# reedrosenbluth/oscen

Hardware: AMD Instinct MI355X
Metric: voices*samples/sec (fm-synth graph, 48 kHz) (higher is better)
Workload: dtype f32

## Files before the change

oscen_amd/csrc/og_cluster.cpp:

```cpp
#include "og_engine.h"

#include <dlfcn.h>
#include <rccl/rccl.h>

#include <condition_variable>
#include <functional>
#include <mutex>
#include <thread>

__global__ void og_bus_accumulate(float* __restrict__ dst, const float* __restrict__ src, size_t n)
{
    const size_t i = (size_t)blockIdx.x * blockDim.x + threadIdx.x;
    if (i < n) dst[i] += src[i];
}

namespace {

struct Rccl {
    void* lib = nullptr;
    ncclResult_t (*CommInitAll)(ncclComm_t*, int, const int*) = nullptr;
    ncclResult_t (*CommDestroy)(ncclComm_t) = nullptr;
    ncclResult_t (*Reduce)(const void*, void*, size_t, ncclDataType_t, ncclRedOp_t, int, ncclComm_t, hipStream_t) = nullptr;
    ncclResult_t (*GroupStart)() = nullptr;
    ncclResult_t (*GroupEnd)() = nullptr;
// ... 373 lines not shown
                    HIPCK(hipStreamWaitEvent(e->stream, free_ev, 0));
                    for (size_t g = 0; g < nf; g += block) {
                        const uint32_t frames = (uint32_t)std::min<size_t>(block, nf - g);
                        e->process_async(frames, buf + g * vc);
                    }
                    e->flush_bus();
                    HIPCK(hipEventRecord(done, e->stream));
                });
            }
            wait_all();
            reduce_and_hand_over(b, nf);
            if (have_prev) {
                HIPCK(hipEventSynchronize(host_ready[b ^ 1]));
                memcpy(out + prev_f0 * channels, h_pin[b ^ 1], prev_nf * channels * sizeof(float));
            }
            have_prev = true;
            prev_f0 = f0;
            prev_nf = nf;
        }
        if (have_prev) {
            HIPCK(hipSetDevice(devs[0]));
            HIPCK(hipEventSynchronize(host_ready[b ^ 1]));
            memcpy(out + prev_f0 * channels, h_pin[b ^ 1], prev_nf * channels * sizeof(float));
        }
        sync_all();
    }
};

extern "C" {

int og_cluster_create(const og_graph_desc* g, uint64_t n_voices_total, const int* device_ids, uint32_t n_shards, og_cluster** out)
{
    if (!g || !device_ids || !out) return set_err(OG_E_INVALID, "null argument");
    if (n_shards == 0 || n_voices_total < n_shards) return set_err(OG_E_INVALID, "need at least one voice per shard");
    return guard([&] {
        std::unique_ptr<og_cluster> c(new og_cluster);
        c->total = n_voices_total;
        for (uint32_t s = 0; s <= n_shards; ++s) c->lo.push_back(n_voices_total * s / n_shards);
        for (uint32_t s = 0; s < n_shards; ++s) {
            const uint64_t nv = c->lo[s + 1] - c->lo[s];
            if (nv > 0xFFFFFFFFull) throw std::runtime_error("more than 2^32 voices in one shard");
            og_engine* raw = nullptr;
            const int rc = og_create(g, (uint32_t)nv, device_ids[s], &raw);
            if (rc != OG_OK) {
                if (rc == OG_E_DEVICE) throw HipError(og_last_error());
                throw std::runtime_error(og_last_error());
            }
            std::unique_ptr<og_engine> e(raw);
            if (e->cg->bus_stage == ogc::BusStage::Convolver)
                throw ogabi::Unsupported("a cluster over a graph with a post-mix Convolver is not supported in this version (the convolver runs on one device's bus)");
            e->bus_stage = false;
            {
                HIPCK(hipSetDevice(e->device));
                e->alloc_bus_buffers(e->auto_batch());
                e->bus_batch = e->auto_batch();
            }
            c->shard.push_back(e.get());
            e.release();
            int di = -1;
            for (size_t d = 0; d < c->devs.size(); ++d)
                if (c->devs[d] == device_ids[s]) di = (int)d;
            if (di < 0) {
                c->devs.push_back(device_ids[s]);
                di = (int)c->devs.size() - 1;
            }
            c->dev_of_shard.push_back(di);
            c->workers.emplace_back(new Worker);
        }
        c->channels = c->shard[0]->cg->channels;
        c->vch = c->shard[0]->cg->voice_channels;
        c->tremolo = c->shard[0]->cg->bus_stage == ogc::BusStage::Tremolo;
        const size_t nd = c->devs.size();
        c->dev_stream.assign(nd, nullptr);
        for (int b = 0; b < 2; ++b) {
            c->sh_buf[b].assign(n_shards, nullptr);
            c->sh_done[b].assign(n_shards, nullptr);
            c->dev_free[b].assign(nd, nullptr);
            c->dev_acc[b].assign(nd, nullptr);
        }
        for (size_t d = 0; d < nd; ++d) {
            HIPCK(hipSetDevice(c->devs[d]));
            HIPCK(hipStreamCreateWithFlags(&c->dev_stream[d], hipStreamNonBlocking));
            for (int b = 0; b < 2; ++b) {
                HIPCK(hipEventCreateWithFlags(&c->dev_free[b][d], hipEventDisableTiming));
                HIPCK(hipEventRecord(c->dev_free[b][d], c->dev_stream[d]));
            }
        }
        for (uint32_t s = 0; s < n_shards; ++s) {
            HIPCK(hipSetDevice(c->shard[s]->device));
            for (int b = 0; b < 2; ++b) HIPCK(hipEventCreateWithFlags(&c->sh_done[b][s], hipEventDisableTiming));
        }
        HIPCK(hipSetDevice(c->devs[0]));
        if (c->tremolo) {
            HIPCK(hipMalloc(&c->d_phase, 4));
            HIPCK(hipMemset(c->d_phase, 0, 4));
        }
        const char* force = ogabi::experiment_knob("OSCEN_GPU_FORCE_RCCL");
        if (nd > 1 || (force && atoi(force) != 0)) {
            Rccl& R = rccl();
            R.load();
            c->comms.assign(nd, nullptr);
            R.ck(R.CommInitAll(c->comms.data(), (int)nd, c->devs.data()), "ncclCommInitAll");
            c->use_rccl = true;
        }
        *out = c.release();
        return OG_OK;
    });
}
// ... 270 lines not shown
```

oscen_amd/csrc/og_engine.cpp:

```cpp
#include "og_engine.h"
#include "og_math.h"
#include "og_bus_conv.hip.h"
#include "og_asset_resample.hip.h"

#define OG_RED_SLICES 64
#define OG_RED_FRAMES 16
static_assert(OG_RED_FRAMES == OG_BUS_CHUNK, "og_bus_reduce reads the chunks og::bus_chunk_reduce writes");
#define OG_RED_GROUP 1024
__device__ __forceinline__ void og_bus_reduce_body(const float* __restrict__ partials, uint32_t n_rows, uint32_t frames,
                                                   float* __restrict__ out, uint32_t out_stride, uint32_t out_off)
{
    __shared__ float part[OG_RED_SLICES][OG_RED_FRAMES];
    __shared__ float quad[OG_RED_SLICES / 4][OG_RED_FRAMES];
    const uint32_t fx = threadIdx.x % OG_RED_FRAMES;
    const uint32_t slice = threadIdx.x / OG_RED_FRAMES;
    const uint32_t f = blockIdx.x * OG_RED_FRAMES + fx;
    const uint32_t row0 = blockIdx.y * OG_RED_GROUP;
    const uint32_t row1 = min(n_rows, row0 + OG_RED_GROUP);
    float acc[8] = {0.0f, 0.0f, 0.0f, 0.0f, 0.0f, 0.0f, 0.0f, 0.0f};
    const float* __restrict__ chunk = partials + (size_t)blockIdx.x * n_rows * OG_RED_FRAMES;
    if (f < frames) {
        uint32_t r = row0 + slice;
        for (; r + 7 * OG_RED_SLICES < row1; r += 8 * OG_RED_SLICES) {
#pragma unroll
// ... 127 lines not shown
    }
    return code;
}
int set_error(int code, const char* m) noexcept
{
    try {
        g_err.assign(m ? m : "");
    } catch (...) {
        g_err.clear();
    }
    return code;
}
}

namespace {
struct DeviceScratch {
    float* p = nullptr;
    explicit DeviceScratch(size_t floats) { HIPCK(hipMalloc(&p, std::max<size_t>(floats, 1) * 4)); }
    ~DeviceScratch() { if (p) (void)hipFree(p); }
    DeviceScratch(const DeviceScratch&) = delete;
    DeviceScratch& operator=(const DeviceScratch&) = delete;
};
std::map<std::string, std::shared_ptr<const SampleData>>& sample_registry()
{
    static std::map<std::string, std::shared_ptr<const SampleData>> R;
    return R;
}
std::mutex& sample_registry_lock()
{
    static std::mutex m;
    return m;
}
}
std::shared_ptr<const SampleData> lookup_sample(const std::string& name)
{
    std::lock_guard<std::mutex> lk(sample_registry_lock());
    auto it = sample_registry().find(name);
    return it == sample_registry().end() ? nullptr : it->second;
}
namespace {
void map_sample_channels(const SampleData& s, uint32_t width, float* dst)
{
    for (size_t t = 0; t < s.frames; ++t)
        for (uint32_t c = 0; c < width; ++c) {
            const uint32_t sc = s.channels == 1 ? 0u : std::min(c, s.channels - 1u);
            dst[t * width + c] = s.interleaved[t * s.channels + sc];
        }
}
}

void og_engine::conv_alloc(size_t need_hist)
{
    const size_t vc = cg->voice_channels;
    const size_t max_frames = (size_t)OG_MAX_BLOCK * batch_cap;
    const size_t keep = std::max(hist_keep, (std::max<size_t>(need_hist, 1) + OG_CONV_S - 1) / OG_CONV_S * OG_CONV_S);
    const size_t len = 2 * keep + 2 * max_frames;
    if (!d_hist || keep != hist_keep || len != hist_len) {
        float* n = nullptr;
        HIPCK(hipMalloc(&n, len * vc * 4));
        HIPCK(hipMemsetAsync(n, 0, len * vc * 4, stream));
        if (d_hist) {
            HIPCK(hipMemcpyAsync(n + (keep - hist_keep) * vc, d_hist + (hist_pos - hist_keep) * vc, hist_keep * vc * 4, hipMemcpyDeviceToDevice, stream));
            HIPCK(hipStreamSynchronize(stream));
            HIPCK(hipFree(d_hist));
        }
        d_hist = n;
        hist_keep = keep;
        hist_len = len;
        hist_pos = keep;
    }
    const uint32_t stride = (uint32_t)((max_frames + 3) / 4 * 4);
    const size_t half = (keep / OG_CONV_S + 1) * vc * stride;
    if (!d_conv_rows || stride != conv_row_stride || half != conv_rows_half) {
        if (d_conv_rows) HIPCK(hipFree(d_conv_rows));
        d_conv_rows = nullptr;
        HIPCK(hipMalloc(&d_conv_rows, 2 * half * 4));
        conv_row_stride = stride;
        conv_rows_half = half;
    }
    HIPCK(hipStreamSynchronize(stream));
}

std::shared_ptr<og_engine::ConvIR> og_engine::conv_build_asset(const std::string& name, const ogc::IrAsset& a)
{
    const uint32_t rate = graph_rate("og_set_bus_ir");
    const bool conform = a.rate != rate;
    const OgResamplePlan plan = conform ? og_resample_plan(a.frames, a.rate, rate) : OgResamplePlan{};
    const uint64_t K = conform ? plan.out_len : a.frames;
    if (K > OG_CONV_MAX_TAPS)
        throw ogabi::Unsupported("impulse response '" + name + "' (" + std::to_string(a.frames) + " frames at " + std::to_string(a.rate) + " Hz) has " +
                                 std::to_string(K) + " taps per channel once conformed to " + std::to_string(rate) + " Hz (at most " + std::to_string(OG_CONV_MAX_TAPS) + ")");
    if (K == 0)
        throw ogabi::Error(OG_E_INVALID, "impulse response '" + name + "' (" + std::to_string(a.frames) + " frames at " + std::to_string(a.rate) + " Hz) is empty once conformed to " + std::to_string(rate) + " Hz");
    const uint32_t vc = cg->voice_channels;
    const bool downmix = vc == 1 && a.channels > 1;
    auto ir = std::make_shared<ConvIR>();
    ir->planes = (a.channels == 1 || vc == 1) ? 1u : vc;
    ir->taps.resize((size_t)ir->planes * K);
    DeviceScratch d_src(a.interleaved.size()), d_conf(conform ? (size_t)K * a.channels : 1);
    bounce.h2d(d_src.p, a.interleaved.data(), a.interleaved.size() * 4, stream);
    if (conform) og_resample_launch(d_src.p, a.frames, a.channels, plan, d_conf.p, stream);
    HIPCK(hipMalloc(&ir->d, ir->taps.size() * 4));
    conv_bufs.push_back(ir->d);
    hipLaunchKernelGGL(og_bus_ir_planes, dim3((unsigned)((K + 255) / 256), ir->planes), dim3(256), 0, stream, conform ? d_conf.p : d_src.p, (uint32_t)K,
                       a.channels, downmix ? 1u : 0u, 1.0f / (float)a.channels, ir->d);
    HIPCK(hipGetLastError());
    bounce.d2h(ir->taps.data(), ir->d, ir->taps.size() * 4, stream);
// ... 175 lines not shown
    }
    TlEvent* sev = h_stage_ev[r];
    uint32_t* upd = h_stage_upd[r];
    const EventTimeline::Batch b = tl.plan_incremental(sev, upd, consumed_horizon(), launch_end());
    if (!b) return false;
    if (b.n_upd == 0) return true;
    HostProf::Scope pc(prof, HostProf::EV_COMMIT);
    tl.commit_incremental(b, sev, upd);
    static_assert(sizeof(OgEvent) == sizeof(uint4), "og_apply_event_updates copies events as 16-byte words");
    const uint32_t n_wg_upd = (uint32_t)((std::max(b.n_upd, b.n_ev) + 255) / 256);
    hipLaunchKernelGGL(og_apply_event_updates, dim3(n_wg_upd), dim3(256), 0, stream, (const uint4*)sev, (uint32_t)b.n_ev,
                       (uint4*)(d_events + b.base), (const uint32_t*)upd, (uint32_t)b.n_upd, d_ev_cursor, d_ev_end);
    HIPCK(hipGetLastError());
    stage_seq[r] = flush_seq + 1;
    batch_staged = true;
    stage_head = (stage_head + 1) % EV_RING;
    return true;
}

void og_engine::upload_events()
{
    if (!tl.needs_upload(launch_end())) return;
    EventTimeline::HoldLocal hold(tl);
    if (!tl.needs_upload(launch_end())) return;
    HostProf::Scope ps(prof, HostProf::SYNC_EVENTS);
    const bool bulk = tl.wants_rebuild() || tl.n_pending() > tl.stage_events() || tl.n_pending() > (size_t)V / 2 + 64 || !d_events;
    if (bulk || !incremental_update()) full_rebuild();
}

bool og_engine::rcp_cover(uint32_t need)
{
    if (need > rcp_cap) return false;
    if (need <= rcp_n) return true;
    const uint32_t n = std::min(rcp_cap, std::max(need, 2 * rcp_n));
    float* t = nullptr;
    HIPCK(hipMalloc(&t, ((size_t)OG_RCP_PAD + n + 1) * sizeof(float)));
    const uint32_t words = OG_RCP_PAD + n + 1;
    hipLaunchKernelGGL(og::rcp_table_fill<0>, dim3((words + 255) / 256), dim3(256), 0, stream, t, n);
    HIPCK(hipGetLastError());
    if (d_rcp) rcp_old.push_back(d_rcp);
    d_rcp = t;
    rcp_n = n;
    return true;
}

void og_engine::alloc_bus_buffers(uint32_t batch)
{
    HIPCK(hipStreamSynchronize(stream));
    for (float** p : {&d_partials, &d_partials2, &d_mono, &d_stage_bus})
        if (*p) {
            HIPCK(hipFree(*p));
            *p = nullptr;
        }
    batch_cap = batch;
    const size_t max_frames = (size_t)OG_MAX_BLOCK * batch;
    const size_t vc = cg->voice_channels;
    HIPCK(hipMalloc(&d_partials, (size_t)n_wg * max_frames * 4 * vc));
    HIPCK(hipMemset(d_partials, 0, (size_t)n_wg * max_frames * 4 * vc));
    HIPCK(hipMalloc(&d_partials2, ((size_t)n_wg / OG_RED_GROUP + 2 + 64) * max_frames * 4));
    HIPCK(hipMalloc(&d_stage_bus, max_frames * OG_MAX_BUS_CHANNELS * 4));
    if (cg->bus_stage == ogc::BusStage::Tremolo) HIPCK(hipMalloc(&d_mono, max_frames * 4));
    if (cg->bus_stage == ogc::BusStage::Convolver) conv_alloc(std::max(conv.cur ? conv.cur->K() : 0u, conv.old ? conv.old->K() : 0u));
    const size_t rows = (size_t)(cg->n_ramps + cg->n_streams);
    for (int i = 0; i < RAMP_RING && rows; ++i) {
        if (d_ramp[i]) HIPCK(hipFree(d_ramp[i]));
        if (h_ramp[i]) HIPCK(hipHostFree(h_ramp[i]));
        d_ramp[i] = h_ramp[i] = nullptr;
        HIPCK(hipMalloc(&d_ramp[i], rows * max_frames * 4));
        HIPCK(hipHostMalloc((void**)&h_ramp[i], rows * max_frames * 4, hipHostMallocDefault));
        ramp_seq[i] = 0;
    }
}

void og_engine::process_async(uint32_t frames, float* d_out)
{
    HIPCK(hipSetDevice(device));
    tl.drop_late_local(frame_now + frames);
    if (!queue.empty() && tl.n_pending() > std::min<size_t>(tl.stage_events() / 2, (size_t)V / 4 + 32)) flush_bus();
    if (queue.empty()) {
        q_frame0 = frame_now;
        q_frames = 0;
        q_ramps = cg->n_streams > 0;
        q_ramp_slot = -1;
    }
    const size_t stride = (size_t)OG_MAX_BLOCK * batch_cap;
    const bool ramping = active_ramps > 0 && cg->n_ramps > 0;
    if ((ramping || cg->n_streams > 0 || q_ramps) && cg->n_ramps + cg->n_streams > 0) {
        if (q_ramp_slot < 0) {
            q_ramp_slot = ramp_head;
            ramp_head = (ramp_head + 1) % RAMP_RING;
            batch_done(ramp_seq[q_ramp_slot]);
            float* tab0 = h_ramp[q_ramp_slot];
            for (size_t i = 0; i < cg->inputs.size(); ++i) {
                const int row = cg->inputs[i].ramp_row;
                if (row >= 0) std::fill(tab0 + (size_t)row * stride, tab0 + (size_t)row * stride + q_frames, ramps[i].current);
            }
        }
        q_ramps = true;
        float* tab = h_ramp[q_ramp_slot];
        for (uint32_t f = 0; f < frames; ++f) {
            for (size_t i = 0; i < cg->inputs.size(); ++i) {
                const int row = cg->inputs[i].ramp_row;
                if (row < 0) continue;
                if (active_ramps > 0 && ramps[i].tick()) active_ramps -= 1;
                tab[(size_t)row * stride + q_frames + f] = ramps[i].current;
            }
        }
        for (size_t i = 0; i < cg->inputs.size(); ++i) {
            if (cg->inputs[i].ramp_row >= 0) values[i] = ramps[i].current;
            const int srow = cg->inputs[i].stream_row;
            for (int k = 0; srow >= 0 && k < std::max(1, cg->inputs[i].decl.channels); ++k)
                memcpy(tab + (size_t)(srow + k) * stride + q_frames, stream_blocks[i].data() + (size_t)k * OG_MAX_BLOCK, (size_t)frames * 4);
        }
    }
    QueuedBlock qb;
    qb.dst = d_out ? d_out : d_bus;
    qb.frames = frames;
    qb.trem_rate = qb.trem_depth = 0.0f;
    qb.conv = 0;
    if (conv_on()) {
        if (conv.old && frame_now >= conv.fade_start + conv_fade_len()) conv_retire(conv.old);
        if (conv_pending) {
            conv_retire(conv.old);
            conv.old = conv.cur;
            conv.old_from = conv.cur_from;
            conv.cur = conv_pending;
            conv.cur_from = conv.fade_start = frame_now;
            conv_pending.reset();
        }
        if (q_conv.empty() || !q_conv.back().same(conv)) q_conv.push_back(conv);
        qb.conv = (uint32_t)q_conv.size() - 1;
    }
    if (cg->bus_stage == ogc::BusStage::Tremolo && bus_stage) {
        ogc::UEnv ev = env();
        qb.trem_rate = cg->tremolo_rate(ev);
        qb.trem_depth = cg->tremolo_depth(ev);
    }
    queue.push_back(qb);
    q_frames += frames;
    frame_now += frames;
    last_frames = frames;
    const bool ramps_done = ramping && active_ramps == 0 && cg->n_streams == 0;
    if (queue.size() >= bus_batch || n_taps > 0 || ramps_done) flush_bus();
}

void og_engine::flush_bus()
{
    if (queue.empty()) return;
    upload_events();
    HostProf::Scope ps(prof, HostProf::LAUNCH);
    OgBlockArgs A;
    memset(&A, 0, sizeof A);
    A.n_voices = V;
    A.frames = q_frames;
    A.ramp_stride = (uint32_t)((size_t)OG_MAX_BLOCK * batch_cap);
    A.lanes = lanes;
    A.split = split;
    A.wide = wide ? 1u : 0u;
    A.frame0 = q_frame0;
    A.state = d_state;
    A.lane_state = d_lane_state;
    A.lane_dump = d_lane_state ? d_lane_state + cg->lane_state.size() * (size_t)V * cg->lpv * cg->lane_width : nullptr;
    A.events = d_events;
    A.ev_end = d_ev_end;
    A.ev_cursor = d_ev_cursor;
    A.partials = d_partials;
    const uint32_t n_chunks16 = (q_frames + OG_RED_FRAMES - 1) / OG_RED_FRAMES;
    A.partial_plane = (uint32_t)((size_t)n_chunks16 * n_wg * OG_RED_FRAMES);
    A.taps = d_taps;
    A.tap_slot = d_tap_slot;
    A.out_ev = d_out_ev;
    A.out_ev_cap = out_ev_cap;
    A.out_ev_count = d_out_ev ? d_out_ev_count : nullptr;
    A.ev_lost = d_out_ev_count ? d_out_ev_count + 1 : nullptr;
    for (size_t k = 0; k < cg->rings.size(); ++k) {
        A.rings[k] = d_ring[k];
        A.ring_cap[k] = ring_cap[k];
    }
    {
        ogc::UEnv e = env();
        uint32_t starts[OG_MAX_LAUNCH_BLOCKS + 1];
        uint32_t acc = 0, nb = 0;
        for (const QueuedBlock& qb : queue) {
            if (nb < OG_MAX_LAUNCH_BLOCKS) starts[nb++] = acc;
            acc += qb.frames;
        }
        e.block_starts = starts;
        e.n_blocks = nb;
        for (const auto& up : cg->uprogs) A.slots[up.dst] = up.fn(e);
    }
    if (cg->player_slot0 >= 0) {
        uint32_t* ps = A.slots + cg->player_slot0;
        ps[0] = (uint32_t)((uintptr_t)d_pool & 0xFFFFFFFFu);
        ps[1] = (uint32_t)((uint64_t)(uintptr_t)d_pool >> 32);
        ps[2] = (uint32_t)((uintptr_t)d_desc & 0xFFFFFFFFu);
        ps[3] = (uint32_t)((uint64_t)(uintptr_t)d_desc >> 32);
        ps[4] = sample_cap;
    }
    if (rcp_cover(release_need(A.slots))) {
        A.rcp_tab = d_rcp;
        A.rcp_len = rcp_n;
    }
    const bool ramps_on = q_ramps && q_ramp_slot >= 0;
    if (ramps_on) {
        const int r = q_ramp_slot;
        const size_t rows = (size_t)(cg->n_ramps + cg->n_streams);
        HIPCK(hipMemcpyAsync(d_ramp[r], h_ramp[r], rows * A.ramp_stride * 4, hipMemcpyHostToDevice, stream));
        ramp_seq[r] = flush_seq + 1;
// ... 1125 lines not shown
    e->tl.reserve_pending(n);
    for (uint32_t i = 0; i < n; ++i)
        e->tl.push(e->phys(voices[i]), std::max(abs_frames[i], e->frame_now), target, values[i], false);
    return OG_OK;
    });
}

int og_process_block_async(og_engine* e, uint32_t frames, float* d_out_bus)
{
    if (!e) return set_err(OG_E_INVALID, "null engine");
    if (!e->inited) return set_err(OG_E_STATE, "og_init must be called before processing");
    if (frames > OG_MAX_BLOCK_SIZE) return set_err(OG_E_INVALID, "frames must be in 0..512");
    return guard([&] {
        if (frames == 0) {
            HIPCK(hipSetDevice(e->device));
            e->flush_bus();
            e->tl.drop_late_local(e->frame_now);
            e->last_frames = 0;
            return OG_OK;
        }
        e->process_async(frames, d_out_bus);
        return OG_OK;
    });
}

int og_process_blocks_async(og_engine* e, uint32_t frames, uint32_t n_blocks, float* d_out_bus, size_t out_stride_bytes)
{
    if (!e) return set_err(OG_E_INVALID, "null engine");
    if (!e->inited) return set_err(OG_E_STATE, "og_init must be called before processing");
    if (frames == 0 || frames > OG_MAX_BLOCK_SIZE) return set_err(OG_E_INVALID, "frames must be in 1..512");
    if (d_out_bus && out_stride_bytes % sizeof(float)) return set_err(OG_E_INVALID, "out_stride_bytes must be a multiple of 4");
    return guard([&] {
        for (uint32_t b = 0; b < n_blocks; ++b)
            e->process_async(frames, d_out_bus ? d_out_bus + (size_t)b * (out_stride_bytes / sizeof(float)) : nullptr);
        return OG_OK;
    });
}

int og_synchronize(og_engine* e)
{
    if (!e) return set_err(OG_E_INVALID, "null engine");
    return guard([&] {
        HIPCK(hipSetDevice(e->device));
        e->flush_bus();
        HIPCK(hipStreamSynchronize(e->stream));
        e->sync_lost_counter();
        return OG_OK;
    });
}

int og_set_bus_batching(og_engine* e, uint32_t blocks)
{
    if (!e) return set_err(OG_E_INVALID, "null engine");
    if (blocks > OG_MAX_LAUNCH_BLOCKS) return set_err(OG_E_INVALID, "bus batching: 0 (automatic) or 1..32 blocks");
    if (blocks == 0) blocks = e->auto_batch();
    return guard([&] {
        HIPCK(hipSetDevice(e->device));
        e->flush_bus();
        if (blocks > e->batch_cap) e->alloc_bus_buffers(blocks);
        e->bus_batch = blocks;
        return OG_OK;
    });
}

int og_flush(og_engine* e)
{
    if (!e) return set_err(OG_E_INVALID, "null engine");
    return guard([&] {
        HIPCK(hipSetDevice(e->device));
        e->flush_bus();
        return OG_OK;
    });
}

int og_process_block(og_engine* e, uint32_t frames, float* out_bus)
{
    if (!e) return set_err(OG_E_INVALID, "null engine");
    if (!e->inited) return set_err(OG_E_STATE, "og_init must be called before processing");
    if (frames > OG_MAX_BLOCK_SIZE) return set_err(OG_E_INVALID, "frames must be in 0..512");
    if (frames == 0 || !out_bus || e->n_taps > 0 || e->blocking_memcpy) {
        int rc = og_process_block_async(e, frames, nullptr);
        if (rc) return rc;
        return guard([&] {
            e->flush_bus();
            if (out_bus && frames)
                e->bounce.d2h(out_bus, e->d_bus, (size_t)frames * e->cg->channels * 4, e->stream);
            HIPCK(hipStreamSynchronize(e->stream));
            return OG_OK;
        });
    }
    return guard([&] {
        HIPCK(hipSetDevice(e->device));
        e->flush_bus();
        if (!e->h_bus_pinned) HIPCK(hipHostMalloc((void**)&e->h_bus_pinned, (size_t)OG_MAX_BLOCK * OG_MAX_BUS_CHANNELS * 4, hipHostMallocDefault));
        e->batch_staged = true;
        const uint64_t seq = e->flush_seq + 1;
        e->process_async(frames, e->h_bus_pinned);
        e->flush_bus();
        e->blocking_waits += 1;
        if (!e->wait_progress(seq)) e->blocking_timeouts += 1;
        memcpy(out_bus, e->h_bus_pinned, (size_t)frames * e->cg->channels * 4);
        return OG_OK;
    });
}

int og_set_stream(og_engine* e, void* s)
{
    if (!e) return set_err(OG_E_INVALID, "null engine");
    return guard([&] {
        HIPCK(hipSetDevice(e->device));
        e->flush_bus();
        HIPCK(hipStreamSynchronize(e->stream));
        if (e->own_stream) HIPCK(hipStreamDestroy(e->stream));
        e->own_stream = false;
        e->stream = (hipStream_t)s;
        return OG_OK;
    });
}

int og_render(og_engine* e, uint64_t total_frames, uint32_t block, float* out_bus)
{
    if (!e || !out_bus) return set_err(OG_E_INVALID, "null argument");
    if (block == 0 || block > OG_MAX_BLOCK_SIZE) return set_err(OG_E_INVALID, "block must be in 1..512");
    if (!e->inited) return set_err(OG_E_STATE, "og_init must be called before processing");
    return guard([&] {
        HIPCK(hipSetDevice(e->device));
        const uint32_t ch = e->cg->channels;
        float* d_all = nullptr;
        HIPCK(hipMalloc(&d_all, (size_t)total_frames * ch * 4));
        e->flush_bus();
        const uint32_t user_batch = e->bus_batch;
        if (e->batch_cap < e->auto_batch()) e->alloc_bus_buffers(e->auto_batch());
        e->bus_batch = e->auto_batch();
        struct Restore {
            og_engine* e;
            uint32_t b;
            ~Restore() { e->bus_batch = b; }
        } restore{e, user_batch};
        try {
            for (uint64_t f0 = 0; f0 < total_frames; f0 += block) {
                const uint32_t frames = (uint32_t)std::min<uint64_t>(block, total_frames - f0);
                e->process_async(frames, d_all + f0 * ch);
            }
            e->flush_bus();
            e->bounce.d2h(out_bus, d_all, (size_t)total_frames * ch * 4, e->stream);
            HIPCK(hipStreamSynchronize(e->stream));
        } catch (...) {
            (void)hipFree(d_all);
            throw;
        }
        HIPCK(hipFree(d_all));
        return OG_OK;
    });
}

int og_set_stream_block(og_engine* e, uint32_t input, const float* samples, uint32_t n)
{
    return ogabi::guard([&]() -> int {
    if (!e || (n && !samples)) return set_err(OG_E_INVALID, "null argument");
    if (input >= e->cg->inputs.size() || e->cg->inputs[input].stream_row < 0) return set_err(OG_E_INVALID, "not a stream input");
    if (n > OG_MAX_BLOCK_SIZE) return set_err(OG_E_INVALID, "a stream block holds at most 512 samples");
    const uint32_t w = (uint32_t)std::max(1, e->cg->inputs[input].decl.channels);
    float* blk = e->stream_blocks[input].data();
    for (uint32_t k = 0; k < w; ++k)
        for (uint32_t j = 0; j < n; ++j) blk[(size_t)k * OG_MAX_BLOCK + j] = samples[(size_t)j * w + k];
    return OG_OK;
    });
}

uint32_t og_num_stream_inputs(const og_engine* e) { return e ? (uint32_t)e->cg->n_stream_inputs : 0; }

uint32_t og_stream_input_channels(const og_engine* e, uint32_t input)
{
    return ogabi::guard_value<uint32_t>((uint32_t)0, [&]() -> uint32_t {
    if (!e || input >= e->cg->inputs.size() || e->cg->inputs[input].stream_row < 0) return 0;
    return (uint32_t)std::max(1, e->cg->inputs[input].decl.channels);
    });
}

int og_render_inputs(og_engine* e, const float* const* inputs, const uint64_t* input_lens, uint32_t n_inputs, uint64_t tail,
                     float* out_bus, uint64_t* frames_rendered)
{
    if (!e || (n_inputs && (!inputs || !input_lens))) return set_err(OG_E_INVALID, "null argument");
    if (!e->inited) return set_err(OG_E_STATE, "og_init must be called before processing");
    if (n_inputs != (uint32_t)e->cg->n_stream_inputs)
        return set_err(OG_E_INVALID, "render: expected " + std::to_string(e->cg->n_stream_inputs) + " input streams, got " + std::to_string(n_inputs));
    uint64_t in_len = 0;
    for (uint32_t i = 0; i < n_inputs; ++i) in_len = std::max(in_len, input_lens[i]);
    const uint64_t total = in_len + tail;
    if (frames_rendered) *frames_rendered = total;
    if (total == 0) return OG_OK;
    if (!out_bus) return set_err(OG_E_INVALID, "null argument");
    return guard([&] {
        HIPCK(hipSetDevice(e->device));
        std::vector<int> sidx;
        for (size_t i = 0; i < e->cg->inputs.size(); ++i)
            if (e->cg->inputs[i].stream_row >= 0) sidx.push_back((int)i);
        const uint32_t ch = e->cg->channels;
        float* d_all = nullptr;
        HIPCK(hipMalloc(&d_all, (size_t)total * ch * 4));
        e->flush_bus();
        const uint32_t user_batch = e->bus_batch;
        if (e->batch_cap < e->auto_batch()) e->alloc_bus_buffers(e->auto_batch());
        e->bus_batch = e->auto_batch();
        struct Restore {
            og_engine* e;
            uint32_t b;
            ~Restore() { e->bus_batch = b; }
        } restore{e, user_batch};
        try {
            for (uint64_t pos = 0; pos < total; pos += OG_MAX_BLOCK) {
                const uint32_t n = (uint32_t)std::min<uint64_t>(OG_MAX_BLOCK, total - pos);
                for (uint32_t k = 0; k < n_inputs; ++k) {
                    float* blk = e->stream_blocks[sidx[k]].data();
                    const uint32_t w = (uint32_t)std::max(1, e->cg->inputs[sidx[k]].decl.channels);
                    for (uint32_t c = 0; c < w; ++c)
                        for (uint32_t j = 0; j < n; ++j)
                            blk[(size_t)c * OG_MAX_BLOCK + j] = (pos + j < input_lens[k]) ? inputs[k][(pos + j) * w + c] : 0.0f;
                }
                e->process_async(n, d_all + pos * ch);
            }
            e->flush_bus();
            e->bounce.d2h(out_bus, d_all, (size_t)total * ch * 4, e->stream);
            HIPCK(hipStreamSynchronize(e->stream));
        } catch (...) {
            (void)hipFree(d_all);
            throw;
        }
        HIPCK(hipFree(d_all));
        return OG_OK;
    });
}

static int find_state_word(const og_engine* e, const char* path)
{
    std::string p;
    for (const char* c = path; *c; ++c) {
        if (*c == '[') p += "__";
        else if (*c != ']' && !isspace((unsigned char)*c)) p.push_back(*c);
    }
    const size_t last = p.rfind('.');
    for (size_t k = 0; k < p.size(); ++k)
        if (p[k] == '.' && k != last) p[k] = '_';
    for (size_t w = 0; w < e->cg->state.size(); ++w)
        if (e->cg->state[w].name == p) return (int)w;
    return -1;
}

int og_state_field_index(const og_engine* e, const char* path)
{
    if (!e || !path) return -1;
    return find_state_word(e, path);
}

int og_read_state_field(og_engine* e, const char* path, uint32_t first_voice, uint32_t n, void* out)
{
// ... 368 lines not shown
```

oscen_amd/csrc/og_engine.h:

```cpp
#pragma once
#include <hip/hip_runtime.h>

#include <algorithm>
#include <cmath>
#include <chrono>
#include <cstdio>
#include <cstdlib>
#include <cstring>
#include <deque>
#include <map>
#include <memory>
#include <mutex>
#include <stdexcept>
#include <string>
#include <unordered_map>
#include <vector>

#include "../../include/oscen_gpu.h"
#include "og_abi.h"
#include "og_graph.h"
#include "og_jit.h"
#include "og_registry.h"
#include "og_timeline.h"

// ... 74 lines not shown
            k ^= 1;
        }
        land(k);
        land(k ^ 1);
    }
    void release()
    {
        for (int i = 0; i < 2; ++i) {
            if (h[i]) (void)hipHostFree(h[i]);
            if (ev[i]) (void)hipEventDestroy(ev[i]);
            h[i] = nullptr;
            ev[i] = nullptr;
        }
    }
};

struct Ramp {
    float current = 0, target = 0, increment = 0;
    uint32_t frames_remaining = 0;
    uint32_t default_frames = 0;
    bool ramping() const { return frames_remaining > 0; }
    void set_immediate(float v)
    {
        current = target = v;
        increment = 0.0f;
        frames_remaining = 0;
    }
    void set_with_ramp(float t, uint32_t frames)
    {
        if (frames == 0) {
            set_immediate(t);
        } else {
            target = t;
            increment = (t - current) / (float)frames;
            frames_remaining = frames;
        }
    }
    bool tick()
    {
        if (frames_remaining > 0) {
            frames_remaining -= 1;
            if (frames_remaining == 0) {
                current = target;
                increment = 0.0f;
                return true;
            }
            current += increment;
        }
        return false;
    }
};

constexpr int RAMP_RING = 8;
constexpr int EV_RING = 8;

struct og_graph_desc {
    ogc::GraphDesc g;
};

struct SampleData {
    std::vector<float> interleaved;
    uint32_t frames = 0, channels = 1;
    uint32_t rate = 0;
};
std::shared_ptr<const SampleData> lookup_sample(const std::string& name);

struct HostProf {
    enum { SYNC_EVENTS, INCREMENTAL, REBUILD, LAUNCH, RAMPS, EV_WAIT, EV_COMMIT, N };
    double t[N] = {};
    uint64_t n[N] = {};
    bool on = ogabi::experiment_knob("OSCEN_GPU_HOST_PROF") != nullptr;
    struct Scope {
        HostProf& p;
        int k;
        std::chrono::steady_clock::time_point t0;
        Scope(HostProf& p_, int k_) : p(p_), k(k_) { if (p.on) t0 = std::chrono::steady_clock::now(); }
        ~Scope()
        {
            if (!p.on) return;
            p.t[k] += std::chrono::duration<double>(std::chrono::steady_clock::now() - t0).count();
            p.n[k] += 1;
        }
    };
    void report() const
    {
        if (!on) return;
        static const char* names[N] = {"sync_events", "incremental_update", "full_rebuild", "flush_bus (launches)", "ramp table",
                                        "  staging-slot wait", "  commit + launch"};
        for (int k = 0; k < N; ++k)
            if (n[k]) fprintf(stderr, "[oscen_gpu host prof] %-22s %9llu calls %10.1f us total %8.2f us/call\n", names[k],
                              (unsigned long long)n[k], t[k] * 1e6, t[k] * 1e6 / (double)n[k]);
    }
};

struct og_engine {
    HostProf prof;
    std::unique_ptr<ogc::CompiledGraph> cg;
    OgLaunchFn launch = nullptr;
    OgZeroLaunchFn launch_zero = nullptr;
    bool zero_spec = true;
    bool last_zero = false;
    OgZeroLaunchFn launch_zero2 = nullptr;
    bool zero2_spec = true;
    bool stage_spec = true;
    bool guards_held = true;
    int last_tier = 0;
// ... 110 lines not shown
        const size_t cap = std::max(need, std::max<size_t>(2 * pool_cap, (size_t)1 << 16));
        float* n = nullptr;
        HIPCK(hipMalloc(&n, cap * 4));
        if (pool_used) HIPCK(hipMemcpyAsync(n, d_pool, pool_used * 4, hipMemcpyDeviceToDevice, stream));
        HIPCK(hipStreamSynchronize(stream));
        if (d_pool) HIPCK(hipFree(d_pool));
        d_pool = n;
        pool_cap = cap;
    }
    void upload_desc()
    {
        const size_t np = cg->players.size();
        if (samples.size() > sample_cap) {
            const uint32_t cap = std::max<uint32_t>(16u, 2u * (uint32_t)samples.size());
            if (d_desc) HIPCK(hipFree(d_desc));
            d_desc = nullptr;
            sample_cap = 0;
            HIPCK(hipMalloc(&d_desc, np * cap * 2 * 4));
            sample_cap = cap;
        }
        std::vector<uint32_t> tab(np * sample_cap * 2, 0u);
        for (size_t k = 0; k < np; ++k)
            for (size_t i = 0; i < samples.size(); ++i) {
                tab[2 * (k * sample_cap + i)] = samples[i].off[cg->players[k].channels];
                tab[2 * (k * sample_cap + i) + 1] = samples[i].pool_frames;
            }
        bounce.h2d(d_desc, tab.data(), tab.size() * 4, stream);
        HIPCK(hipStreamSynchronize(stream));
    }
    uint32_t load_sample(const std::string& name, const SampleData& sd);
    int find_player(const char* node) const
    {
        std::string p;
        for (const char* c = node; *c; ++c) {
            if (*c == '[') p += "__";
            else if (*c == '.') p.push_back('_');
            else if (*c != ']' && !isspace((unsigned char)*c)) p.push_back(*c);
        }
        for (size_t k = 0; k < cg->players.size(); ++k)
            if (cg->players[k].name == p) return (int)k;
        return -1;
    }
    OgEvent* d_events = nullptr;
    uint32_t* d_ev_end = nullptr;
    uint32_t* d_ev_cursor = nullptr;
    float* d_partials = nullptr;
    float* d_partials2 = nullptr;
    float* d_rcp = nullptr;
    uint32_t rcp_n = 0;
    uint32_t rcp_cap = OG_RCP_MAX;
    std::vector<float*> rcp_old;
    std::vector<uint32_t> tap_voices;
    uint32_t bus_batch = 1;
    uint32_t batch_cap = 1;
    struct QueuedBlock {
        float* dst;
        uint32_t frames;
        float trem_rate, trem_depth;
        uint32_t conv;
    };
    std::vector<QueuedBlock> queue;
    uint64_t q_frame0 = 0;
    uint32_t q_frames = 0;
    bool q_ramps = false;
    int q_ramp_slot = -1;
    float* d_stage_bus = nullptr;
    float* d_bus = nullptr;
    float* d_ramp[RAMP_RING] = {};
    float* h_ramp[RAMP_RING] = {};
    uint64_t ramp_seq[RAMP_RING] = {};
    int ramp_head = 0;
    OgOutEvent* d_out_ev = nullptr;
    uint32_t* d_out_ev_count = nullptr;
    uint32_t out_ev_cap = 0;
    uint64_t out_ev_overflow = 0;
    uint64_t ev_lost_total = 0;
    std::vector<OgOutEvent> out_ev_carry;
    float* d_taps = nullptr;
    int32_t* d_tap_slot = nullptr;
    uint32_t n_taps = 0;
    uint32_t last_frames = 0;

    EventTimeline tl;
    std::vector<uint32_t> phys_of, logical_of;
    uint32_t phys(uint32_t v) const { return phys_of.empty() ? v : phys_of[v]; }
    uint32_t logical(uint32_t p) const { return logical_of.empty() ? p : logical_of[p]; }
    uint64_t launch_end() const { return queue.empty() ? frame_now : q_frame0 + q_frames; }
    void sync_lost_counter();
    TlEvent* h_stage_ev[EV_RING] = {};
    uint32_t* h_stage_upd[EV_RING] = {};
    uint32_t* d_stage_upd[EV_RING] = {};
    uint64_t stage_seq[EV_RING] = {};
    uint64_t flush_seq = 0;
    bool batch_staged = false;
    volatile uint64_t* h_progress = nullptr;
    float* h_bus_pinned = nullptr;
    bool blocking_memcpy = false;
    uint64_t blocking_waits = 0, blocking_timeouts = 0;
    bool wait_progress(uint64_t seq)
    {
        using clk = std::chrono::steady_clock;
        const auto t0 = clk::now();
        auto next_query = t0 + std::chrono::microseconds(256);
        for (uint32_t spins = 0; !h_progress || *h_progress < seq; ++spins) {
            if ((spins & 255u) == 255u) {
                const auto now = clk::now();
                if (now >= next_query) {
// ... 2 lines not shown
                    if (q != hipErrorNotReady) HIPCK(q);
                    next_query = now + std::chrono::microseconds(128);
                }
            }
#if defined(__x86_64__)
            __builtin_ia32_pause();
#endif
        }
        return true;
    }
    bool batch_done(uint64_t seq)
    {
        if (seq == 0 || (h_progress && *h_progress >= seq)) return true;
        if (seq > flush_seq) return true;
        HIPCK(hipStreamSynchronize(stream));
        return true;
    }
    int stage_head = 0;
    uint32_t bus_passes = 0;
    uint64_t frame_now = 0;

    bool bus_stage = true;

    bool timing = false;
    std::vector<hipEvent_t> t_start, t_stop;
    unsigned long long* h_clock = nullptr;
    static constexpr size_t T_CLOCK = 8192;
    size_t t_used = 0;
    size_t t_blocks = 0;
    double last_clock_ghz = 0.0;

    ~og_engine();

    ogc::UEnv env() const { return ogc::UEnv{sr, values.data()}; }

    void upload_initial_state();
    size_t ring_bytes() const
    {
        size_t n = 0;
        for (size_t k = 0; k < cg->rings.size(); ++k) n += (size_t)ring_cap[k] * V * 4;
        return n;
    }

    void reset_timeline()
    {
        tl.reset();
        HIPCK(hipMemsetAsync(d_ev_cursor, 0, (size_t)V * 4, stream));
        HIPCK(hipMemsetAsync(d_ev_end, 0, (size_t)V * 4, stream));
    }

    uint32_t auto_batch() const
    {
        const size_t per_block = (size_t)std::max<uint32_t>(n_wg, 1u) * 256u * 4u;
        const size_t b = ((size_t)32 << 20) / per_block;
        return (uint32_t)std::min<size_t>(OG_MAX_LAUNCH_BLOCKS, std::max<size_t>(8, b));
    }
    uint64_t consumed_horizon() const { return queue.empty() ? frame_now : q_frame0; }
    void full_rebuild();
    bool incremental_update();
    void upload_events();

    uint32_t release_need(const uint32_t* slots) const
    {
        uint32_t need = 0;
        for (int k : cg->release_slots) need = std::max(need, slots[k]);
        return need;
    }
    bool rcp_cover(uint32_t need);
    void alloc_bus_buffers(uint32_t batch);
    void process_async(uint32_t frames, float* d_out);
    void flush_bus();
    static void launch_bus_tremolo(const float* mono, uint32_t frames, float rate, float depth, float sr, float* phase_state, float* out,
                                   hipStream_t stream);
};
```

oscen_amd/csrc/og_graph.cpp:

```cpp
#include "og_graph.h"
#include "og_rt_digest.h"

#include <algorithm>
#include <cctype>
#include <cmath>
#include <cstdio>
#include <cstdlib>
#include <cstring>
#include <deque>
#include <set>
#include <sstream>
#include <stdexcept>

namespace ogc {
std::string normalize_type(const std::string& type);

uint64_t fnv1a(const std::string& s)
{
    uint64_t h = 1469598103934665603ull;
    for (unsigned char c : s) {
        h ^= c;
        h *= 1099511628211ull;
    }
    return h;
// ... 4867 lines not shown
    for (int zs : out.zero2_slots) z2desc << " " << zs;
    z2desc << " hold +-0,\n// slot(s)";
    for (int fs : out.finite_slots) z2desc << " " << fs;
    z2desc << " are finite and no ramp ticks.  Left out or folded:";
    for (const NodeInst& n : cg.nodes)
        if (zset.count(n.id) || z2set.count(n.id)) z2desc << " " << n.decl->name;
    z2desc << ".";
    if (out.stage_spec)
        z2desc << "\n// Its four-wave pipeline has the stage-uniform envelope bodies of og_stage_uniform.hip.h (digest " << OG_STAGEU_DIGEST
               << "); uniform slot 159 switches them off.";
    std::ostringstream pre;
    if (out.lpv > 1) pre << "\n#define OG_HPL " << out.lane_width << " // harmonics per lane (OGC_HPL)";
    if (cg.ev_capacity != 2) pre << "\n#define OG_NODE_EVENTS_PER_FRAME " << cg.ev_capacity << " // event_queue_capacity of a node type of this graph";
    pre << "\n#include \"og_kernel_rt.hip.h\"\n#include \"og_nodes.hip.h\"\n" << (cg.uses_adsrp ? "#include \"og_adsr_params.hip.h\"\n" : "")
        << (out.players.empty() ? "" : "#include \"og_sample_player.hip.h\"\n") << "\n"
        << "#if OG_NODE_EVENTS_PER_FRAME <= 4\n#define OG_EV_LOOP_PRAGMA _Pragma(\"unroll\")\n#else\n#define OG_EV_LOOP_PRAGMA _Pragma(\"unroll 1\")\n#endif\n"
        << "#define SF(i) og::slot_f(A, (i))\n#define SU(i) og::slot_u(A, (i))\n"
        << "#define RV(row, slot) (RAMPS ? A.ramp_table[(size_t)(row) * A.ramp_stride + f] : og::slot_f(A, (slot)))\n"
        << "#define ST(row) A.ramp_table[(size_t)(row) * A.ramp_stride + f]\n"
        << "// the pipelined kernels: the chunk's rows are in rv_<row>[] when the chunk body is the unrolled one (BoolC::pre)\n"
        << "#define RVP(row, slot) (RAMPS ? og::row_pick<decltype(chk)::pre>(rv_##row, j, A, (row), f) : og::slot_f(A, (slot)))\n"
        << "#define STP(row) og::row_pick<decltype(chk)::pre>(rv_##row, j, A, (row), f)\n\n";
    const std::string ns = std::string("og_gen_") + hs;
    write_unit_head(units[0].os, g.name, desc.str(), pre.str(), ns, out.lpv, gen.body);
    if (units[1].on) write_unit_head(units[1].os, g.name, zdesc.str(), pre.str(), ns + "_z", out.lpv, zbody);
    if (units[2].on)
        write_unit_head(units[2].os, g.name, z2desc.str(), pre.str(), ns + "_z2", out.lpv, z2body,
                        out.stage_spec ? "#include \"og_stage_uniform.hip.h\"\n" : "");

    const char* variants[4][3] = {{"00", "false", "false"}, {"10", "true", "false"}, {"01", "false", "true"},
                                  {"11", "true", "true"}};
    int waves_eu = (out.lpv > 1 && out.lane_width == 8) ? 3 : 4;
    {
        int player_channels = 0;
        for (const auto& pl : out.players) player_channels += pl.channels;
        if (player_channels > 2) waves_eu = 2;
    }
    auto shape = [&](const std::string& kp, const std::string& fn, int threads, const std::string& attr, const std::string& zattr, const std::string& extra) {
        for (Unit& u : units)
            for (auto& v : variants)
                if (u.on && !(u.sfx && v[1][0] != 'f'))
                    write_kernel_entry(u.os, threads, u.sfx ? zattr : attr, kp + hs + "_" + v[0] + (u.sfx ? u.sfx : ""), ns + u.tail() + "::" + fn,
                                       std::string(u.sfx ? "false" : v[1]) + ", " + v[2] + extra);
    };
    const std::string budget = " __attribute__((amdgpu_waves_per_eu(" + std::to_string(waves_eu) + ")))";
    shape("og_k_", "voice_block", 64, budget, budget, "");
    std::vector<std::pair<int, int>> depths;
    if (!cg.groups2.empty()) depths.push_back({2, (int)cg.groups2.size()});
    if (!cg.groups4.empty()) depths.push_back({4, (int)cg.groups4.size()});
    for (auto [K, W] : depths) {
        const std::string zbudget = K == 4 ? " __attribute__((amdgpu_waves_per_eu(6)))" : "";
        shape("og_k" + std::to_string(K) + "_", "voice_block_p" + std::to_string(K), 64 * W, "", zbudget, "");
    }
    if (out.wide4) shape("og_k4w_", "voice_block_p4", 64 * (int)cg.groups4.size(), "", "", ", " + wide_args);

    for (Unit& u : units)
        if (u.on)
            u.os << "\n#ifndef OG_JIT\n#include \"og_registry.h\"\n"
                 << "static void og_launch_" << hs << u.tail() << "(const OgBlockArgs& A, " << (u.sfx ? "" : "bool ramps, ") << "bool taps, hipStream_t s)\n{\n"
                 << "    const dim3 grid(((size_t)A.n_voices * " << out.lpv << " + A.lanes - 1) / A.lanes), block(OG_WAVE);\n";
    auto branch = [&](const std::string& cond, size_t waves, const std::string& kp) {
        for (Unit& u : units) {
            if (!u.on) continue;
            u.os << "    if (" << cond << "\n"
                 << "        const dim3 gk((A.n_voices + OG_WAVE - 1) / OG_WAVE), bk(" << waves << " * OG_WAVE);\n";
            write_dispatch(u.os, "        ", kp + hs, u.sfx, "gk, bk");
            u.os << "        return;\n    }\n";
        }
    };
    if (out.wide4) branch("A.split == 4u && A.wide) { // four waves per 64 voices, 16-frame hand-offs", cg.groups4.size(), "og_k4w_");
    for (auto [K, W] : depths)
        branch("A.split == " + std::to_string(K) + "u) { // " + std::to_string(W) + " waves per 64 voices", (size_t)W, "og_k" + std::to_string(K) + "_");
    for (Unit& u : units) {
        if (!u.on) continue;
        write_dispatch(u.os, "    ", std::string("og_k_") + hs, u.sfx, "grid, block");
        u.os << "}\n";
        if (u.sfx)
            u.os << "static const OgZeroKernelRegistrar og_" << u.sfx << "reg_" << hs << "(0x" << hs << "ull, &og_launch_" << hs << u.tail()
                 << (!strcmp(u.sfx, "z2") ? ", 2" : "") << ");\n#endif\n";
    }
    std::ostringstream& src = units[0].os;
    src << "static int og_occ_" << hs << "(int depth) // resident workgroups per CU of each shape (registers, LDS)\n{\n    int n = 0;\n";
    for (auto [K, W] : depths)
        src << "    if (depth == " << K << ") { (void)hipOccupancyMaxActiveBlocksPerMultiprocessor(&n, og_k" << K << "_" << hs << "_00, " << 64 * W
            << ", 0); return n; }\n";
    if (out.wide4)
        src << "    if (depth == 5) { (void)hipOccupancyMaxActiveBlocksPerMultiprocessor(&n, og_k4w_" << hs << "_00, " << 64 * (int)cg.groups4.size()
            << ", 0); return n; } // (5 = the wide four-wave form)\n";
    src << "    if (depth <= 1) (void)hipOccupancyMaxActiveBlocksPerMultiprocessor(&n, og_k_" << hs << "_00, OG_WAVE, 0);\n    return n;\n}\n"
        << "static const OgKernelRegistrar og_reg_" << hs << "(0x" << hs << "ull, \"" << g.name << "\", &og_launch_"
        << hs << ", &og_occ_" << hs << ");\n#endif\n";
    out.source = units[0].os.str();
    out.zero_source = units[1].os.str();
    out.zero2_source = units[2].os.str();
}

}

std::unique_ptr<CompiledGraph> compile(const GraphDesc& g_in)
{
    const auto gen = lower(g_in, nullptr);
    CompiledGraph& out = *gen->out;
    std::set<int> zset = find_zero_chain(*gen);
    const std::string zbody = lower_variant(g_in, zset, out);
    if (zbody.empty()) {
        zset.clear();
// ... 21 lines not shown
```

oscen_amd/csrc/og_graph.h:

```cpp
#pragma once
#include "og_abi.h"
#include <cstdint>
#include <functional>
#include <map>
#include <memory>
#include <string>
#include <vector>

namespace ogc {

enum class Kind { Value = 0, Event = 1, Stream = 2 };

enum class Rate {
    Const = 0,
    UBlock = 1,
    UFrame = 2,
    VBlock = 3,
    Vary = 4,
};

struct UEnv {
    float sample_rate;
    const float* input_values;
    const uint32_t* block_starts = nullptr;
// ... 42 lines not shown
struct PolyInfo {
    bool is_wrapper = false;
    uint32_t declared_voices = 0;
    std::string voice_type;
    std::string frequency_input;
    std::string gate_input;
    std::string midi_input;
    std::vector<std::string> dropped_event_outputs;
};
GraphDesc lower_poly_wrapper(const GraphDesc& g, PolyInfo* info = nullptr);
std::map<std::string, GraphDesc> builtin_voice_graph_types();

struct InputInfo {
    GInput decl;
    int slot = -1;
    int ramp_row = -1;
    int state_word = -1;
    int event_index = -1;
    int stream_row = -1;
};
struct StateWord {
    std::string name;
    bool is_float = true;
    std::function<uint32_t(const UEnv&)> init;
    bool read_mostly = false;
};
struct UniformProg {
    int dst;
    std::function<uint32_t(const UEnv&)> fn;
};
struct RingSpec {
    std::string name;
    float rate_factor = 1.0f;
    uint32_t capacity(float graph_sr) const;
};
enum class BusStage { None = 0, Tremolo = 1, Convolver = 2 };
struct CompiledGraph {
    std::string name;
    std::string source;
    std::string zero_source;
    std::string zero2_source;
    uint64_t hash = 0;
    std::vector<InputInfo> inputs;
    std::vector<StateWord> state;
    std::vector<StateWord> lane_state;
    std::vector<RingSpec> rings;
    struct PlayerSpec {
        std::string name;
        int channels = 1;
        int sample_word = -1, playhead_word = -1;
    };
    std::vector<PlayerSpec> players;
    int player_slot0 = -1;
    int lpv = 1;
    int lane_width = 1;
    bool can_split = false;
    int max_pipeline = 1;
    bool wide4 = false;
    std::vector<int> zero_slots;
    std::vector<int> zero2_slots, finite_slots;
    bool stage_spec = false;
    int valu_estimate = 0;
    BusStage bus_stage = BusStage::None;
    HostFn tremolo_rate, tremolo_depth;
    std::string bus_ir_name;
    std::shared_ptr<const std::vector<float>> bus_ir;
    std::vector<UniformProg> uprogs;
    std::vector<int> release_slots;
    int n_slots = 0;
    int n_ramps = 0;
    int n_streams = 0;
    int n_stream_inputs = 0;
    int n_event_inputs = 0;
    std::vector<std::string> event_outputs;
    bool has_node_event_outputs = false;
    uint32_t channels = 1;
    uint32_t voice_channels = 1;
    struct OutChan {
        std::string name;
        int offset, width;
    };
    std::vector<OutChan> output_channels;
    uint32_t latency_samples = 0;
    std::vector<std::string> node_order;
    std::vector<std::string> schedule_order;
    int find_input(const std::string& n) const;
};

std::unique_ptr<CompiledGraph> compile(const GraphDesc& g);
void check_reference_rules(const GraphDesc& g);

struct UserPort {
    std::string name;
    Kind kind = Kind::Stream;
    float def = 0.0f;
    int arg = -1;
    int channels = 1;
};
struct UserState {
    std::string name;
    bool is_uint = false;
    float init_f = 0.0f;
    uint32_t init_u = 0;
    int arg = -1;
};
struct UserNodeType {
// ... 59 lines not shown
```

Before: 875.9 billion.

## Allow deeper bus-batch queues for wide graphs with frame-based launch cap

After: 925.3 billion, median of 6. 1.06x the previous value.

```diff
diff --git a/oscen_amd/csrc/og_cluster.cpp b/oscen_amd/csrc/og_cluster.cpp
--- a/oscen_amd/csrc/og_cluster.cpp
+++ b/oscen_amd/csrc/og_cluster.cpp
@@ -449,8 +449,9 @@
             e->bus_stage = false;
             {
                 HIPCK(hipSetDevice(e->device));
-                e->alloc_bus_buffers(e->auto_batch());
-                e->bus_batch = e->auto_batch();
+                const uint32_t shard_batch = std::min<uint32_t>(e->auto_batch(), OG_MAX_LAUNCH_BLOCKS);
+                e->alloc_bus_buffers(shard_batch);
+                e->bus_batch = shard_batch;
             }
             c->shard.push_back(e.get());
             e.release();
diff --git a/oscen_amd/csrc/og_engine.cpp b/oscen_amd/csrc/og_engine.cpp
--- a/oscen_amd/csrc/og_engine.cpp
+++ b/oscen_amd/csrc/og_engine.cpp
@@ -203,7 +203,7 @@
 void og_engine::conv_alloc(size_t need_hist)
 {
     const size_t vc = cg->voice_channels;
-    const size_t max_frames = (size_t)OG_MAX_BLOCK * batch_cap;
+    const size_t max_frames = cap_frames;
     const size_t keep = std::max(hist_keep, (std::max<size_t>(need_hist, 1) + OG_CONV_S - 1) / OG_CONV_S * OG_CONV_S);
     const size_t len = 2 * keep + 2 * max_frames;
     if (!d_hist || keep != hist_keep || len != hist_len) {
@@ -485,8 +485,8 @@
             HIPCK(hipFree(*p));
             *p = nullptr;
         }
-    batch_cap = batch;
-    const size_t max_frames = (size_t)OG_MAX_BLOCK * batch;
+    cap_frames = launch_frames_cap(batch);
+    const size_t max_frames = cap_frames;
     const size_t vc = cg->voice_channels;
     HIPCK(hipMalloc(&d_partials, (size_t)n_wg * max_frames * 4 * vc));
     HIPCK(hipMemset(d_partials, 0, (size_t)n_wg * max_frames * 4 * vc));
@@ -510,13 +510,14 @@
     HIPCK(hipSetDevice(device));
     tl.drop_late_local(frame_now + frames);
     if (!queue.empty() && tl.n_pending() > std::min<size_t>(tl.stage_events() / 2, (size_t)V / 4 + 32)) flush_bus();
+    if (!queue.empty() && (size_t)q_frames + frames > cap_frames) flush_bus();
     if (queue.empty()) {
         q_frame0 = frame_now;
         q_frames = 0;
         q_ramps = cg->n_streams > 0;
         q_ramp_slot = -1;
     }
-    const size_t stride = (size_t)OG_MAX_BLOCK * batch_cap;
+    const size_t stride = cap_frames;
     const bool ramping = active_ramps > 0 && cg->n_ramps > 0;
     if ((ramping || cg->n_streams > 0 || q_ramps) && cg->n_ramps + cg->n_streams > 0) {
         if (q_ramp_slot < 0) {
@@ -586,7 +587,7 @@
     memset(&A, 0, sizeof A);
     A.n_voices = V;
     A.frames = q_frames;
-    A.ramp_stride = (uint32_t)((size_t)OG_MAX_BLOCK * batch_cap);
+    A.ramp_stride = (uint32_t)cap_frames;
     A.lanes = lanes;
     A.split = split;
     A.wide = wide ? 1u : 0u;
@@ -1818,12 +1819,16 @@
 int og_set_bus_batching(og_engine* e, uint32_t blocks)
 {
     if (!e) return set_err(OG_E_INVALID, "null engine");
-    if (blocks > OG_MAX_LAUNCH_BLOCKS) return set_err(OG_E_INVALID, "bus batching: 0 (automatic) or 1..32 blocks");
+    if (blocks > OG_MAX_QUEUE_BLOCKS)
+        return set_err(OG_E_INVALID, "bus batching: 0 (automatic) or 1.." + std::to_string(OG_MAX_QUEUE_BLOCKS) + " blocks");
+    if (blocks > OG_MAX_LAUNCH_BLOCKS && e->cg->reads_block_starts)
+        return set_err(OG_E_INVALID, "bus batching: a graph whose event handlers read frame_offset takes 0 (automatic) or 1.." +
+                                         std::to_string(OG_MAX_LAUNCH_BLOCKS) + " blocks");
     if (blocks == 0) blocks = e->auto_batch();
     return guard([&] {
         HIPCK(hipSetDevice(e->device));
         e->flush_bus();
-        if (blocks > e->batch_cap) e->alloc_bus_buffers(blocks);
+        if (e->launch_frames_cap(blocks) > e->cap_frames) e->alloc_bus_buffers(blocks);
         e->bus_batch = blocks;
         return OG_OK;
     });
@@ -1896,7 +1901,7 @@
         HIPCK(hipMalloc(&d_all, (size_t)total_frames * ch * 4));
         e->flush_bus();
         const uint32_t user_batch = e->bus_batch;
-        if (e->batch_cap < e->auto_batch()) e->alloc_bus_buffers(e->auto_batch());
+        if (e->cap_frames < e->launch_frames_cap(e->auto_batch())) e->alloc_bus_buffers(e->auto_batch());
         e->bus_batch = e->auto_batch();
         struct Restore {
             og_engine* e;
@@ -1967,7 +1972,7 @@
         HIPCK(hipMalloc(&d_all, (size_t)total * ch * 4));
         e->flush_bus();
         const uint32_t user_batch = e->bus_batch;
-        if (e->batch_cap < e->auto_batch()) e->alloc_bus_buffers(e->auto_batch());
+        if (e->cap_frames < e->launch_frames_cap(e->auto_batch())) e->alloc_bus_buffers(e->auto_batch());
         e->bus_batch = e->auto_batch();
         struct Restore {
             og_engine* e;
diff --git a/oscen_amd/csrc/og_engine.h b/oscen_amd/csrc/og_engine.h
--- a/oscen_amd/csrc/og_engine.h
+++ b/oscen_amd/csrc/og_engine.h
@@ -150,6 +150,8 @@
 };
 
 constexpr int RAMP_RING = 8;
+constexpr uint32_t OG_MAX_QUEUE_BLOCKS = 256;
+constexpr size_t OG_WIDE_ROW_BUDGET = (size_t)256 << 20;
 constexpr int EV_RING = 8;
 
 struct og_graph_desc {
@@ -366,7 +368,7 @@
     std::vector<float*> rcp_old;
     std::vector<uint32_t> tap_voices;
     uint32_t bus_batch = 1;
-    uint32_t batch_cap = 1;
+    size_t cap_frames = OG_MAX_BLOCK;
     struct QueuedBlock {
         float* dst;
         uint32_t frames;
@@ -475,8 +477,20 @@
     uint32_t auto_batch() const
     {
         const size_t per_block = (size_t)std::max<uint32_t>(n_wg, 1u) * 256u * 4u;
+        if (wide && !cg->reads_block_starts && cg->bus_stage != ogc::BusStage::Convolver) {
+            const size_t b = OG_WIDE_ROW_BUDGET / (per_block * std::max<size_t>(cg->voice_channels, 1));
+            return (uint32_t)std::min<size_t>(OG_MAX_QUEUE_BLOCKS, std::max<size_t>(8, b));
+        }
         const size_t b = ((size_t)32 << 20) / per_block;
         return (uint32_t)std::min<size_t>(OG_MAX_LAUNCH_BLOCKS, std::max<size_t>(8, b));
+    }
+    size_t launch_frames_cap(uint32_t blocks) const
+    {
+        if (blocks <= OG_MAX_LAUNCH_BLOCKS) return (size_t)OG_MAX_BLOCK * blocks;
+        size_t f = std::max<size_t>(OG_MAX_LAUNCH_FRAMES, (size_t)256 * blocks);
+        const size_t plane = (size_t)0xFFFFFFFFu / std::max<uint32_t>(n_wg, 1u) / OG_BUS_CHUNK * OG_BUS_CHUNK;
+        if (cg->voice_channels > 1) f = std::max<size_t>(OG_MAX_LAUNCH_FRAMES, std::min(f, plane));
+        return f;
     }
     uint64_t consumed_horizon() const { return queue.empty() ? frame_now : q_frame0; }
     void full_rebuild();
diff --git a/oscen_amd/csrc/og_graph.cpp b/oscen_amd/csrc/og_graph.cpp
--- a/oscen_amd/csrc/og_graph.cpp
+++ b/oscen_amd/csrc/og_graph.cpp
@@ -4943,6 +4943,7 @@
         const std::string zbudget = K == 4 ? " __attribute__((amdgpu_waves_per_eu(6)))" : "";
         shape("og_k" + std::to_string(K) + "_", "voice_block_p" + std::to_string(K), 64 * W, "", zbudget, "");
     }
+    out.reads_block_starts = cg.blk_slot0 >= 0;
     if (out.wide4) shape("og_k4w_", "voice_block_p4", 64 * (int)cg.groups4.size(), "", "", ", " + wide_args);
 
     for (Unit& u : units)
diff --git a/oscen_amd/csrc/og_graph.h b/oscen_amd/csrc/og_graph.h
--- a/oscen_amd/csrc/og_graph.h
+++ b/oscen_amd/csrc/og_graph.h
@@ -118,6 +118,7 @@
     };
     std::vector<PlayerSpec> players;
     int player_slot0 = -1;
+    bool reads_block_starts = false;
     int lpv = 1;
     int lane_width = 1;
     bool can_split = false;
```
